# panagiotou23/model-predictive-control

Hardware: AMD Instinct MI355X
Metric: MPC solves/sec, bicycle model N=20 nx=4 nu=2, batch=65536; 1/2/4/8 GPU (higher is better)
Workload: dtype f64

## Files before the change

model_predictive_control_amd/csrc/mpc_device.hpp:

```cpp
#pragma once
#include <hip/hip_runtime.h>
#include <stdint.h>

namespace mpc {

constexpr int KIN = 0;
constexpr int PAC = 1;

struct DevCfg {
    int model, N, S, nfe, wrap_mode, clip_inputs, constr_mode, sm;
    int nx, n, m, M;
    int max_iter, max_outer, hess_heuristic, max_no_progress;
    int max_num_initial_retries, max_num_retries, max_total_num_retries, max_total_inner, max_total_evals;
    int no_spec;
    int chain;
    int all_rows;
    int no_memo;
    int no_la;
    double h;
    double v_ref;
    double w[6];
    double lf, lr, mass, inv_mass, inv_iz;
    double bf, cf, df, br, cr, dr, cm1, cm2, cr0, cr2;
    double accel, friction, max_drive, max_steer;
// ... 150 lines not shown
#pragma clang fp contract(off)
    const double kf = rint(x * 6.36619772367581382433e-01);
    double r = fma(-kf, 1.57079632679489655800e+00, x);
    r = fma(-kf, 6.12323399573676603587e-17, r);
    r = fma(-kf, -1.49738490485916983294e-33, r);
    const int q = (int)kf;
    const SinCos k = kernel_sincos(r);
    const double sn = k.s, cs = k.c;
    SinCos o;
    const bool swap = q & 1;
    const double sv = swap ? cs : sn, cv = swap ? sn : cs;
    o.s = (q & 2) ? -sv : sv;
    o.c = ((q + 1) & 2) ? -cv : cv;
    return o;
}

__device__ __forceinline__ SinCos rotate_sincos(const SinCos &a, double d)
{
#pragma clang fp contract(off)
    const SinCos k = kernel_sincos(d);
    SinCos o;
    o.s = fma(a.c, k.s, a.s * k.c);
    o.c = fma(-a.s, k.s, a.c * k.c);
    return o;
}

__device__ __noinline__ SinCos sincos_any(double x)
{
    const SinCos slow = ocml_sincos(x);
    const SinCos fast = lean_sincos(fabs(x) < 1.0e5 ? x : 0.0);
    return fabs(x) < 1.0e5 ? fast : slow;
}
__device__ __forceinline__ SinCos m_sincos(double x)
{
    if (__builtin_expect(__ballot(!(fabs(x) < 1.0e5)) == 0ull, 1)) return lean_sincos(x);
    return sincos_any(x);
}
__device__ __forceinline__ double m_sin(double x) { return m_sincos(x).s; }

__device__ __forceinline__ double atan_reduced(double r, double off_hi, double off_lo)
{
#pragma clang fp contract(off)
    const double z = r * r, w = z * z;
    double s1 = fma(w, 1.62858201153657823623e-02, 4.97687799461593236017e-02);
    s1 = fma(w, s1, 6.66107313738753120669e-02);
    s1 = fma(w, s1, 9.09088713343650656196e-02);
    s1 = fma(w, s1, 1.42857142725034663711e-01);
    s1 = z * fma(w, s1, 3.33333333333329318027e-01);
    double s2 = fma(w, -3.65315727442169155270e-02, -5.83357013379057348645e-02);
    s2 = fma(w, s2, -7.69187620504482999495e-02);
    s2 = fma(w, s2, -1.11111104054623557880e-01);
    s2 = w * fma(w, s2, -1.99999999998764832476e-01);
    return off_hi - ((r * (s1 + s2) - off_lo) - r);
}

__device__ __forceinline__ double atan_ratio(double ay, double ax)
{
#pragma clang fp contract(off)
    const bool lo = ay <= 0.41421356237309503 * ax;
    const bool hi = ay > 2.4142135623730951 * ax;
    const double num = lo ? ay : (hi ? -ax : ay - ax);
    const double den = lo ? ax : (hi ? ay : ay + ax);
    const double r = num / den;
    const double off_hi = lo ? 0.0 : (hi ? 1.57079632679489655800e+00 : 7.85398163397448278999e-01);
    const double off_lo = lo ? 0.0 : (hi ? 6.12323399573676603587e-17 : 3.06161699786838301793e-17);
    return atan_reduced(r, off_hi, off_lo);
}

MPC_ATAN_FN double m_atan(double x)
{
    const double a = fabs(x);
#ifndef MPC_ATAN_ALWAYS_DIVIDES
    if (__builtin_expect(__ballot(!(a <= 0.41421356237309503)) == 0ull, 1)) return copysign(atan_reduced(a, 0.0, 0.0), x);
#endif
    const double t = a < 1.0e300 ? atan_ratio(a, 1.0) : 1.57079632679489655800e+00;
    return x != x ? x : copysign(t, x);
}

MPC_ATAN_FN double lean_atan2(double y, double x)
{
#pragma clang fp contract(off)
    double t = atan_ratio(fabs(y), fabs(x));
    if (signbit(x)) t = 3.14159265358979311600e+00 - (t - 1.22464679914735317720e-16);
    return copysign(t, y);
}
__device__ __forceinline__ double m_atan2(double y, double x)
{
    const double ay = fabs(y), ax = fabs(x);
    const bool ok = ay < 1.0e300 && ax < 1.0e300 && (ay != 0.0 || ax != 0.0);
    if (__builtin_expect(__ballot(!ok) == 0ull, 1)) return lean_atan2(y, x);
    const double slow = ocml_atan2(y, x);
    const double fast = lean_atan2(ok ? y : 1.0, ok ? x : 1.0);
    return ok ? fast : slow;
}

template <int MODEL> struct StageInput;

template <> struct StageInput<KIN> {
    double ad;
    double beta;
    double sb_lr;
    double cb_lr;
    double dbeta;
    double mk0, mk1;
};
template <> struct StageInput<PAC> {
    double d, dl, sd, cd;
    double mk0, mk1;
};

MPC_DEV void clip_input(const DevCfg &c, double &d, double &dl, double &mk0, double &mk1)
{
    mk0 = 1.0; mk1 = 1.0;
    if (c.clip_inputs) {
        if (d > c.max_drive) { d = c.max_drive; mk0 = 0.0; }
        else if (d < -c.max_drive) { d = -c.max_drive; mk0 = 0.0; }
        if (dl > c.max_steer) { dl = c.max_steer; mk1 = 0.0; }
        else if (dl < -c.max_steer) { dl = -c.max_steer; mk1 = 0.0; }
    }
}

MPC_DEV void prep_input(const DevCfg &c, double d, double dl, StageInput<KIN> &s)
{
#pragma clang fp contract(off)
    clip_input(c, d, dl, s.mk0, s.mk1);
    const double L = c.lf + c.lr;
    const bool ok = fabs(dl) <= 0.75 && L > 0.0;
    SinCos sd = kernel_sincos(ok ? dl : 0.0);
    bool mid = false;
    if (__builtin_expect(__ballot(!ok) != 0ull, 0)) {
        mid = !ok && fabs(dl) < 1.0e5 && L > 0.0;
        const SinCos sr = lean_sincos(mid ? dl : 0.0);
        sd.s = mid ? sr.s : sd.s; sd.c = mid ? sr.c : sd.c;
    }
    const bool fast = ok || mid;
    double td = sd.s / sd.c;
    double t = c.lf * td;
    const double hyp2 = t * t + L * L;
    const double rh = 1.0 / sqrt(hyp2);
    double sb = t * rh, cb = L * rh;
    double beta;
    if (__builtin_expect(__ballot(!fast) == 0ull, 1)) beta = lean_atan2(t, L);
    else {
        const double td_s = m_tan(dl), t_s = c.lf * td_s;
        const double beta_s = m_atan2(t_s, L);
        const SinCos scb = m_sincos(beta_s);
        const double beta_f = lean_atan2(fast ? t : 0.0, fast ? L : 1.0);
        beta = fast ? beta_f : beta_s;
        td = fast ? td : td_s; t = fast ? t : t_s;
        sb = fast ? sb : scb.s; cb = fast ? cb : scb.c;
    }
    s.beta = beta;
    s.sb_lr = sb / c.lr;
    s.cb_lr = cb / c.lr;
    s.dbeta = (L / (t * t + L * L)) * c.lf * (1.0 + td * td);
    s.ad = c.accel * d;
}

MPC_DEV void prep_input(const DevCfg &c, double d, double dl, StageInput<PAC> &s)
{
    clip_input(c, d, dl, s.mk0, s.mk1);
    s.d = d; s.dl = dl;
    const SinCos sc = m_sincos(dl);
    s.sd = sc.s; s.cd = sc.c;
}

template <int MODEL> struct Lin;
template <> struct Lin<KIN> { double s, co, v; };
template <> struct Lin<PAC> {
    double sp, cp, f0, f1;
    double vx, vy, om;
    double ffy, Df, Dr;
    double vx_r1, a1_r1, vx_r2, a2_r2;
};

template <bool LIN>
MPC_DEV void rhs(const DevCfg &c, const StageInput<KIN> &u, const double (&x)[4], double (&k)[4],
                 Lin<KIN> &lin)
{
    const SinCos sc = m_sincos(x[2] + u.beta);
    const double s = sc.s, co = sc.c;
    const double v = x[3];
    k[0] = v * co;
    k[1] = v * s;
    k[2] = v * u.sb_lr;
    k[3] = u.ad - c.friction * v;
    if (LIN) { lin.s = s; lin.co = co; lin.v = v; }
}

template <bool LIN>
MPC_DEV void rhs_sc(const DevCfg &c, const StageInput<KIN> &u, const double (&x)[4], const SinCos &sc,
                    double (&k)[4], Lin<KIN> &lin)
{
#pragma clang fp contract(off)
    const double s = sc.s, co = sc.c;
    const double v = x[3];
    k[0] = v * co;
    k[1] = v * s;
    k[2] = v * u.sb_lr;
    k[3] = u.ad - c.friction * v;
    if (LIN) { lin.s = s; lin.co = co; lin.v = v; }
}

struct StepTrig { SinCos sc[4]; };
MPC_DEV void step_trig(const DevCfg &c, const StageInput<KIN> &u, const double (&x)[4], StepTrig &tr)
{
#pragma clang fp contract(off)
    const double h = c.h, hh = 0.5 * h;
    const double v1 = x[3];
    const double v2 = v1 + hh * (u.ad - c.friction * v1);
    const double v3 = v1 + hh * (u.ad - c.friction * v2);
    const double d2 = hh * (v1 * u.sb_lr), d3 = hh * (v2 * u.sb_lr), d4 = h * (v3 * u.sb_lr);
    const double th = x[2] + u.beta;
    const bool ok = fabs(d2) <= 0.75 && fabs(d3) <= 0.75 && fabs(d4) <= 0.75 && fabs(th) < 1.0e5;
    if (__builtin_expect(__ballot(!ok) == 0ull, 1)) {
        tr.sc[0] = lean_sincos(th);
        tr.sc[1] = rotate_sincos(tr.sc[0], d2);
        tr.sc[2] = rotate_sincos(tr.sc[0], d3);
        tr.sc[3] = rotate_sincos(tr.sc[0], d4);
    } else {
        const double ths = ok ? th : 0.0;
        StepTrig f;
        f.sc[0] = lean_sincos(ths);
        f.sc[1] = rotate_sincos(f.sc[0], ok ? d2 : 0.0);
        f.sc[2] = rotate_sincos(f.sc[0], ok ? d3 : 0.0);
        f.sc[3] = rotate_sincos(f.sc[0], ok ? d4 : 0.0);
        const SinCos g0 = m_sincos(th), g1 = m_sincos((x[2] + d2) + u.beta);
        const SinCos g2 = m_sincos((x[2] + d3) + u.beta), g3 = m_sincos((x[2] + d4) + u.beta);
        tr.sc[0] = ok ? f.sc[0] : g0; tr.sc[1] = ok ? f.sc[1] : g1;
        tr.sc[2] = ok ? f.sc[2] : g2; tr.sc[3] = ok ? f.sc[3] : g3;
    }
}

MPC_DEV void vjp(const DevCfg &c, const StageInput<KIN> &u, const Lin<KIN> &l, const double (&w)[4],
                 double (&yb)[4], double (&ub)[2])
{
    const double A = l.v * (w[1] * l.co - w[0] * l.s);
    yb[0] = 0.0; yb[1] = 0.0;
    yb[2] = A;
    yb[3] = w[0] * l.co + w[1] * l.s + w[2] * u.sb_lr - w[3] * c.friction;
    const double beta_b = A + w[2] * l.v * u.cb_lr;
    ub[0] += w[3] * c.accel * u.mk0;
    ub[1] += beta_b * u.dbeta * u.mk1;
}

MPC_DEV double sign_of(double v) { return (v > 0.0 ? 1.0 : 0.0) - (v < 0.0 ? 1.0 : 0.0); }

MPC_DEV void pac_assemble(const DevCfg &c, const StageInput<PAC> &u, double vx, double vy, double om, double sp,
                          double cp, double stf, double str, double (&k)[6])
{
#pragma clang fp contract(off)
    const double frx = (c.cm1 - c.cm2 * vx) * u.d - c.cr0 * sign_of(vx) - c.cr2 * vx * vx;
    const double ffy = c.df * stf;
    const double fry = c.dr * str;
    k[0] = vx * cp - vy * sp;
    k[1] = vx * sp + vy * cp;
    k[2] = om;
    k[3] = (frx - ffy * u.sd + c.mass * vy * om) * c.inv_mass;
    k[4] = (fry + ffy * u.cd - c.mass * vx * om) * c.inv_mass;
    k[5] = (ffy * c.lf * u.cd - fry * c.lr) * c.inv_iz;
}

template <bool LIN>
MPC_DEV void rhs(const DevCfg &c, const StageInput<PAC> &u, const double (&x)[6], double (&k)[6],
                 Lin<PAC> &lin)
{
    const double vx = x[3], vy = x[4], om = x[5];
    const double a1 = om * c.lf + vy;
    const double a2 = om * c.lr - vy;
    const double fa1 = fabs(a1), fa2 = fabs(a2), fvx = fabs(vx);
    const bool ok = fabs(x[2]) < 1.0e5 && fa1 < 1.0e300 && fa2 < 1.0e300 && fvx < 1.0e300 &&
                    (fvx != 0.0 || (fa1 != 0.0 && fa2 != 0.0)) && fabs(u.dl) < 1.0e5 &&
                    fabs(c.cf) < 6.0e4 && fabs(c.cr) < 6.0e4;
    double sp, cp, af, ar, stf, ctf, str, ctr;
    if (__builtin_expect(__ballot(!ok) == 0ull, 1)) {
        const SinCos scp = lean_sincos(x[2]);
        sp = scp.s; cp = scp.c;
        af = u.dl - lean_atan2(a1, vx);
        ar = lean_atan2(a2, vx);
        const SinCos a = lean_sincos(c.cf * m_atan(c.bf * af)), b = lean_sincos(c.cr * m_atan(c.br * ar));
        stf = a.s; ctf = a.c; str = b.s; ctr = b.c;
    } else {
        const SinCos scp = m_sincos(x[2]);
        sp = scp.s; cp = scp.c;
        af = u.dl - m_atan2(a1, vx);
        ar = m_atan2(a2, vx);
        const SinCos a = m_sincos(c.cf * m_atan(c.bf * af)), b = m_sincos(c.cr * m_atan(c.br * ar));
        stf = a.s; ctf = a.c; str = b.s; ctr = b.c;
    }
    const double ffy = c.df * stf;
    pac_assemble(c, u, vx, vy, om, sp, cp, stf, str, k);
    if (LIN) {
        lin.sp = sp; lin.cp = cp; lin.f0 = k[0]; lin.f1 = k[1];
        lin.vx = vx; lin.vy = vy; lin.om = om;
        lin.ffy = ffy;
        const double baf = c.bf * af, bar = c.br * ar;
        lin.Df = c.df * ctf * c.cf * c.bf / (1.0 + baf * baf);
        lin.Dr = c.dr * ctr * c.cr * c.br / (1.0 + bar * bar);
        const double ir1 = 1.0 / (a1 * a1 + vx * vx), ir2 = 1.0 / (a2 * a2 + vx * vx);
        lin.vx_r1 = vx * ir1; lin.a1_r1 = a1 * ir1;
        lin.vx_r2 = vx * ir2; lin.a2_r2 = a2 * ir2;
    }
}

MPC_DEV void vjp(const DevCfg &c, const StageInput<PAC> &u, const Lin<PAC> &l, const double (&w)[6],
                 double (&yb)[6], double (&ub)[2])
// ... 621 lines not shown
```

model_predictive_control_amd/csrc/mpc_eval.hpp:

```cpp
#pragma once
#include "mpc_solver.hpp"

#ifndef MPC_K1B_WAVES_PAC
#define MPC_K1B_WAVES_PAC 1
#endif
#ifndef MPC_QUAD_WAVES
#define MPC_QUAD_WAVES 2
#endif

namespace mpc {

struct SlotMap {
    int nG, nC, gpad, nblk_g, nblk;
    __device__ SlotMap(const int *counts, int nG_imm, int nC_imm)
    {
        nG = counts ? counts[0] : nG_imm;
        nC = counts ? counts[1] : nC_imm;
        gpad = (nG + 63) & ~63;
        nblk_g = gpad >> 6;
        nblk = nblk_g + ((nC + 63) >> 6);
    }
};

template <int MODEL, bool PA = false>
__global__ void __launch_bounds__(64, 2)
rollout_kernel(const DevCfg c, const WsArg<PA> w, const int *__restrict__ lists,
               const int *__restrict__ counts, int nG_imm, int nC_imm)
{
    constexpr int NX = ModelDim<MODEL>::NX;
    extern __shared__ double lds[];
    double *tile = lds;
    int *s_agent = (int *)(lds + 64 * (c.n + 1));
    const SlotMap sm(counts, nG_imm, nC_imm);
    const int sb = blockIdx.x;
    if (sb >= sm.nblk) return;
    const int lane = threadIdx.x;
    const bool is_g = sb < sm.nblk_g;
    const int uslot = sb * 64 + lane;
    const int kslot = is_g ? uslot : uslot - sm.gpad;
    const bool active = kslot < (is_g ? sm.nG : sm.nC);
    const int *list = counts ? (is_g ? lists : lists + w.Ls) : nullptr;
    const int raw = active ? (list ? list[kslot] : kslot) : -1;
    const int a = raw < 0 ? -1 : raw & AGENT_MASK;
    const int n = c.n, N = c.N, ld = n + 1;
    s_agent[lane] = raw;
    w.agent_of[uslot] = raw;
    __syncthreads();
    const int total = 64 * n;
    for (int base = 0; base < total; base += 64 * 8) {
        double v[8];
        int off[8];
#pragma unroll
        for (int u = 0; u < 8; u++) {
            const int idx = base + u * 64 + lane;
            const int r = idx / n, j = idx - r * n;
            const int ar = idx < total ? s_agent[r] : -1;
            off[u] = ar >= 0 ? r * ld + j : -1;
            v[u] = ar >= 0 ? ((ar & CH2_BIT) ? w.xe2 : w.xe)[(size_t)(ar & AGENT_MASK) * n + j] : 0.0;
        }
#pragma unroll
        for (int u = 0; u < 8; u++) if (off[u] >= 0) tile[off[u]] = v[u];
    }
    __syncthreads();
    if (!active) return;
    DevCfg cm_;
    if constexpr (PA) { cm_ = c; agent_cfg(cm_, w.ptab, w.pidx, a); }
    const DevCfg &cm = PA ? cm_ : c;
    const size_t St = (size_t)w.St;
    const double *urow = tile + lane * ld;
    double x[NX];
#pragma unroll
    for (int i = 0; i < NX; i++) { x[i] = w.x0[(size_t)a * NX + i]; w.trajx[(size_t)i * St + uslot] = x[i]; }
    for (int k = 0; k < N; k++) {
        const double d = urow[2 * k], dl = urow[2 * k + 1];
        w.useq[(size_t)(2 * k) * St + uslot] = d;
        w.useq[(size_t)(2 * k + 1) * St + uslot] = dl;
        StageInput<MODEL> u;
        prep_input(cm, d, dl, u);
        stage_forward<MODEL>(cm, u, x);
#pragma unroll
        for (int i = 0; i < NX; i++) w.trajx[(size_t)((k + 1) * NX + i) * St + uslot] = x[i];
    }
}

#ifndef MPC_K1A_WAVES
#define MPC_K1A_WAVES 3
#endif
template <class Put>
__device__ __forceinline__ void kin_wide_rollout(const DevCfg &c, const double (&x0)[4], double d, double dl, int lane, Put put);
template <bool PA = false>
__global__ void __launch_bounds__(64, MPC_K1A_WAVES)
rollout_pair_kernel(const DevCfg c, const WsArg<PA> w, const int *__restrict__ lists,
                    const int *__restrict__ counts, int nG_imm, int nC_imm)
{
#pragma clang fp contract(off)
#if MPC_DEV_STAMP == 1
    DevStamp stamp(blockIdx.x);
#endif
    constexpr int RPB = 32;
    extern __shared__ double lds[];
    const SlotMap sm(counts, nG_imm, nC_imm);
    const int lane = threadIdx.x, q = lane >> 1, half = lane & 1;
    const int uslot = blockIdx.x * RPB + q;
    const int nslots = sm.nblk * 64;
    const bool is_g = uslot < sm.gpad;
    const int kslot = is_g ? uslot : uslot - sm.gpad;
    const bool active = uslot < nslots && kslot < (is_g ? sm.nG : sm.nC);
    const int *list = counts ? (is_g ? lists : lists + w.Ls) : nullptr;
    const int raw = active ? (list ? list[kslot] : kslot) : -1;
    const int n = c.n, N = c.N, ld = n + 1;
    if (half == 0 && uslot < nslots) w.agent_of[uslot] = raw;
    if (__ballot(active) == 0ull) return;
    {
        const double *__restrict__ row = ((raw & CH2_BIT) ? w.xe2 : w.xe) + (size_t)(raw & AGENT_MASK) * n;
        for (int j0 = half; j0 < n; j0 += 16) {
            double v[8];
#pragma unroll
            for (int t = 0; t < 8; t++) v[t] = active && j0 + 2 * t < n ? row[j0 + 2 * t] : 0.0;
#pragma unroll
            for (int t = 0; t < 8; t++) if (j0 + 2 * t < n) lds[q * ld + j0 + 2 * t] = v[t];
        }
    }
    __builtin_amdgcn_wave_barrier();
    const int a = active ? raw & AGENT_MASK : 0;
    DevCfg cm_;
    if constexpr (PA) { cm_ = c; if (active) agent_cfg(cm_, w.ptab, w.pidx, a); }
    const DevCfg &cm = PA ? cm_ : c;
    const size_t St = (size_t)w.St;
    const double *urow = lds + q * ld;
    double x[4];
#pragma unroll
    for (int i = 0; i < 4; i++) x[i] = active ? w.x0[(size_t)a * 4 + i] : 0.0;
    bool redo = false;
    auto put = [&](int k) {
        if (!active || redo) return;
        w.trajx[(size_t)(k * 4 + 2 * half) * St + uslot] = half ? x[2] : x[0];
        w.trajx[(size_t)(k * 4 + 2 * half + 1) * St + uslot] = half ? x[3] : x[1];
    };
    put(0);
    auto stage = [&](int k, const StageInput<KIN> &u) {
        const double d = urow[2 * k], dl = urow[2 * k + 1];
        if (active) w.useq[(size_t)(2 * k + half) * St + uslot] = half ? dl : d;
        redo = redo || !kin4_in_range(cm, u, x);
#if MPC_DEV_STAMP == 1
        if (__ballot(redo) != 0ull) stamp.nfall++;
#endif
        double ph = x[2], v = x[3];
        KinRK k0, k1, k2, k3;
        const double ph0 = ph; kin_rk(cm, u, v, k0); kin_next(cm, k0, ph, v);
        const double ph1 = ph; kin_rk(cm, u, v, k1); kin_next(cm, k1, ph, v);
        const double ph2 = ph; kin_rk(cm, u, v, k2); kin_next(cm, k2, ph, v);
        const double ph3 = ph; kin_rk(cm, u, v, k3); kin_next(cm, k3, ph, v);
        KinRK ka, kb;
        ka.v1 = half ? k2.v1 : k0.v1; ka.v2 = half ? k2.v2 : k0.v2; ka.v3 = half ? k2.v3 : k0.v3; ka.v4 = half ? k2.v4 : k0.v4;
        ka.kp1 = half ? k2.kp1 : k0.kp1; ka.kp2 = half ? k2.kp2 : k0.kp2; ka.kp3 = half ? k2.kp3 : k0.kp3;
        kb.v1 = half ? k3.v1 : k1.v1; kb.v2 = half ? k3.v2 : k1.v2; kb.v3 = half ? k3.v3 : k1.v3; kb.v4 = half ? k3.v4 : k1.v4;
        kb.kp1 = half ? k3.kp1 : k1.kp1; kb.kp2 = half ? k3.kp2 : k1.kp2; kb.kp3 = half ? k3.kp3 : k1.kp3;
        double dxa, dya, dxb, dyb;
        kin_increment(cm, u, half ? ph2 : ph0, ka, !redo, dxa, dya);
        kin_increment(cm, u, half ? ph3 : ph1, kb, !redo, dxb, dyb);
        const double oxa = dpp_xchg<0xB1>(dxa), oya = dpp_xchg<0xB1>(dya);
        const double oxb = dpp_xchg<0xB1>(dxb), oyb = dpp_xchg<0xB1>(dyb);
        double px = x[0], py = x[1];
        px = px + dxa; py = py + dya;
        px = px + dxb; py = py + dyb;
        px = px + oxa; py = py + oya;
        px = px + oxb; py = py + oyb;
        x[0] = px; x[1] = py; x[2] = ph; x[3] = v;
        put(k + 1);
    };
    for (int k = 0; k < N; k += 2) {
        const int km = min(k + half, N - 1);
        StageInput<KIN> um, up;
#if MPC_DEV_STAMP == 1
        if (__ballot(!(fabs(urow[2 * km + 1]) <= 0.75)) != 0ull) stamp.nmid++;
        if (__ballot(!(fabs(urow[2 * km + 1]) < 1.0e5)) != 0ull) stamp.nslow++;
#endif
        prep_input(cm, urow[2 * km], urow[2 * km + 1], um);
        up.ad = dpp_xchg<0xB1>(um.ad); up.beta = dpp_xchg<0xB1>(um.beta);
        up.sb_lr = dpp_xchg<0xB1>(um.sb_lr); up.cb_lr = dpp_xchg<0xB1>(um.cb_lr);
        up.dbeta = dpp_xchg<0xB1>(um.dbeta); up.mk0 = dpp_xchg<0xB1>(um.mk0); up.mk1 = dpp_xchg<0xB1>(um.mk1);
        StageInput<KIN> ua, ub;
        ua.ad = half ? up.ad : um.ad; ua.beta = half ? up.beta : um.beta; ua.sb_lr = half ? up.sb_lr : um.sb_lr;
        ua.cb_lr = half ? up.cb_lr : um.cb_lr; ua.dbeta = half ? up.dbeta : um.dbeta;
        ua.mk0 = half ? up.mk0 : um.mk0; ua.mk1 = half ? up.mk1 : um.mk1;
        ub.ad = half ? um.ad : up.ad; ub.beta = half ? um.beta : up.beta; ub.sb_lr = half ? um.sb_lr : up.sb_lr;
        ub.cb_lr = half ? um.cb_lr : up.cb_lr; ub.dbeta = half ? um.dbeta : up.dbeta;
        ub.mk0 = half ? um.mk0 : up.mk0; ub.mk1 = half ? um.mk1 : up.mk1;
        stage(k, ua);
        if (k + 1 < N) stage(k + 1, ub);
    }
    unsigned long long todo = __ballot(redo && active && half == 0);
    while (todo != 0ull) {
        const int l0 = (int)__builtin_ctzll(todo);
        todo &= todo - 1ull;
        const int aq = __builtin_amdgcn_readlane(raw, l0) & AGENT_MASK;
        const int uq = blockIdx.x * RPB + (l0 >> 1);
        const double *uro = lds + (l0 >> 1) * ld;
        const bool stage_lane = lane < N;
        const double dq = stage_lane ? uro[2 * lane] : 0.0, dlq = stage_lane ? uro[2 * lane + 1] : 0.0;
        double xq[4];
#pragma unroll
        for (int i = 0; i < 4; i++) xq[i] = w.x0[(size_t)aq * 4 + i];
        double *const tj = w.trajx + uq;
        if constexpr (PA) {
            DevCfg cq = c;
            agent_cfg_uniform(cq, w.ptab, w.pidx, aq);
            kin_wide_rollout(cq, xq, dq, dlq, lane, [=](int k, int i, double v) { tj[(size_t)(k * 4 + i) * St] = v; });
        } else
        kin_wide_rollout(c, xq, dq, dlq, lane, [=](int k, int i, double v) { tj[(size_t)(k * 4 + i) * St] = v; });
    }
}


template <bool PA = false>
__global__ void __launch_bounds__(64, MPC_QUAD_WAVES)
rollout_quad_kernel(const DevCfg c, const WsArg<PA> w, const int *__restrict__ lists,
                    const int *__restrict__ counts, int nG_imm, int nC_imm)
{
    constexpr int NX = 6, RPB = 16;
    extern __shared__ double lds[];
#if MPC_DEV_STAMP == 4
    DevStamp stamp(blockIdx.x);
#endif
    const SlotMap sm(counts, nG_imm, nC_imm);
    const int lane = threadIdx.x, q = lane >> 2, role = lane & 3;
    const int uslot = blockIdx.x * RPB + q;
    const int nslots = sm.nblk * 64;
    const bool is_g = uslot < sm.gpad;
    const int kslot = is_g ? uslot : uslot - sm.gpad;
    const bool active = uslot < nslots && kslot < (is_g ? sm.nG : sm.nC);
    const int *list = counts ? (is_g ? lists : lists + w.Ls) : nullptr;
    const int raw = active ? (list ? list[kslot] : kslot) : -1;
    const int n = c.n, N = c.N, ld = n + 1;
    if (role == 0 && uslot < nslots) w.agent_of[uslot] = raw;
    if (active) {
        const double *__restrict__ row = ((raw & CH2_BIT) ? w.xe2 : w.xe) + (size_t)(raw & AGENT_MASK) * n;
        for (int j0 = role; j0 < n; j0 += 32) {
            double v[8];
#pragma unroll
            for (int t = 0; t < 8; t++) v[t] = j0 + 4 * t < n ? row[j0 + 4 * t] : 0.0;
#pragma unroll
            for (int t = 0; t < 8; t++) if (j0 + 4 * t < n) lds[q * ld + j0 + 4 * t] = v[t];
        }
    }
    __builtin_amdgcn_wave_barrier();
    if (!active) return;
    const int a = raw & AGENT_MASK;
    DevCfg cm_;
    if constexpr (PA) { cm_ = c; agent_cfg(cm_, w.ptab, w.pidx, a); }
    const DevCfg &cm = PA ? cm_ : c;
    const size_t St = (size_t)w.St;
    const double *urow = lds + q * ld;
    double x[NX];
#pragma unroll
    for (int i = 0; i < NX; i++) x[i] = w.x0[(size_t)a * NX + i];
    auto put = [&](int k) {
        w.trajx[(size_t)(k * NX + role) * St + uslot] = role == 0 ? x[0] : role == 1 ? x[1] : role == 2 ? x[2] : x[3];
        if (role < 2) w.trajx[(size_t)(k * NX + 4 + role) * St + uslot] = role == 0 ? x[4] : x[5];
    };
    put(0);
    for (int k = 0; k < N; k++) {
        const double d = urow[2 * k], dl = urow[2 * k + 1];
        if (role == 0) w.useq[(size_t)(2 * k) * St + uslot] = d;
        if (role == 1) w.useq[(size_t)(2 * k + 1) * St + uslot] = dl;
        StageInput<PAC> u;
        prep_input(cm, d, dl, u);
#if MPC_DEV_STAMP == 4
        {
            bool fin = true;
#pragma unroll
            for (int i = 0; i < NX; i++) fin = fin && fabs(x[i]) < 1.0e300;
            const bool inr = fabs(x[2]) < 1.0e5 && fabs(dl) < 1.0e5 && (x[3] != 0.0 || (x[5] * c.lf + x[4] != 0.0 && x[5] * c.lr - x[4] != 0.0));
            if (__ballot(!fin) != 0ull) stamp.nfall++;
            if (__ballot(fin && !inr) != 0ull) stamp.nmid++;
            if (__ballot(!fin) != 0ull && k == 0) stamp.nslow++;
        }
#endif
        stage_forward_quad(cm, u, x, role);
        put(k + 1);
    }
}

template <class Put>
__device__ __forceinline__ void kin_wide_rollout(const DevCfg &c, const double (&x0)[4], double d, double dl, int lane, Put put)
{
    const int N = c.N;
    const bool stage_lane = lane < N;
    StageInput<KIN> u;
    prep_input(c, d, dl, u);
    if (lane == 0) {
#pragma unroll
        for (int i = 0; i < 4; i++) put(0, i, x0[i]);
    }
    double ph = x0[2], v = x0[3];
    constexpr int PASS = 4;
    double cph[PASS] = {0.0, 0.0, 0.0, 0.0}, cv[PASS] = {0.0, 0.0, 0.0, 0.0}, eph = 0.0, ev = 0.0;
    int gen = 0;
    bool anygen = false;
#pragma unroll
    for (int p = 0; p < PASS; p++) {
        const int k1 = N < 16 * (p + 1) ? N : 16 * (p + 1);
        for (int k = 16 * p; k < k1; k++) {
            StageInput<KIN> uk;
            uk.ad = rdlane(u.ad, k); uk.beta = rdlane(u.beta, k); uk.sb_lr = rdlane(u.sb_lr, k);
            const double xs[4] = {0.0, 0.0, ph, v};
            const bool inr = __ballot(!kin4_in_range(c, uk, xs)) == 0ull;
            anygen = anygen || !inr;
#pragma unroll
            for (int j = 0; j < 4; j++) {
                if (lane == ((4 * k + j) & 63)) { cph[p] = ph; cv[p] = v; gen |= inr ? 0 : 1 << p; }
                KinRK kr;
                if (inr) { kin_rk(c, uk, v, kr); kin_next(c, kr, ph, v); }
                else { kin_gen_rk(c, uk, v, kr); kin_gen_next(c, kr, ph, v); }
            }
            if (lane == k) { eph = ph; ev = v; }
        }
    }
    double dx[PASS] = {0.0, 0.0, 0.0, 0.0}, dy[PASS] = {0.0, 0.0, 0.0, 0.0};
#pragma unroll
    for (int p = 0; p < PASS; p++) {
        const int s = 64 * p + lane;
        if (64 * p >= 4 * N) break;
        const int k = (s >> 2) < N ? (s >> 2) : N - 1;
        StageInput<KIN> uk;
        uk.ad = __shfl(u.ad, k); uk.beta = __shfl(u.beta, k); uk.sb_lr = __shfl(u.sb_lr, k);
        const bool g = ((gen >> p) & 1) != 0 && (s >> 2) < N;
        KinRK kr;
        kin_rk(c, uk, cv[p], kr);
        kin_increment(c, uk, cph[p], kr, !g, dx[p], dy[p]);
        if (anygen) {
            double gx, gy;
            kin_gen_rk(c, uk, g ? cv[p] : 0.0, kr);
            kin_gen_increment(c, uk, g ? cph[p] : 0.0, g ? cv[p] : 0.0, kr, gx, gy);
            dx[p] = g ? gx : dx[p]; dy[p] = g ? gy : dy[p];
        }
    }
    double px = x0[0], py = x0[1], epx = 0.0, epy = 0.0;
#pragma unroll
    for (int p = 0; p < PASS; p++) {
        const int k0 = 16 * p, k1 = N < 16 * (p + 1) ? N : 16 * (p + 1);
        for (int k = k0; k < k1; k++) {
#pragma clang fp contract(off)
#pragma unroll
            for (int j = 0; j < 4; j++) {
                px = px + rdlane(dx[p], (4 * k + j) & 63);
                py = py + rdlane(dy[p], (4 * k + j) & 63);
            }
            if (lane == k) { epx = px; epy = py; }
        }
    }
    if (stage_lane) { put(lane + 1, 0, epx); put(lane + 1, 1, epy); put(lane + 1, 2, eph); put(lane + 1, 3, ev); }
}

template <bool PA = false>
__global__ void __launch_bounds__(256)
rollout_wide_kernel(const DevCfg c, const WsArg<PA> w, const int *__restrict__ lists,
                    const int *__restrict__ counts)
{
    const SlotMap sm(counts, 0, 0);
    const int lane = threadIdx.x & 63, wv = threadIdx.x >> 6;
    const int uslot = blockIdx.x * 4 + wv;
    if (uslot >= sm.nblk * 64) return;
// ... 396 lines not shown
```

model_predictive_control_amd/csrc/mpc_solver.hpp:

```cpp
#pragma once
#include "mpc_device.hpp"
#include <float.h>

namespace mpc {

constexpr int REC = 64;
enum {
    R_PSI, R_L, R_GAMMA, R_PHI, R_PSIXH, R_PP, R_GP, R_TAU, R_PSIN, R_LN, R_GAMMAN, R_PSIXHN, R_GPN,
    R_PPN, R_SIGPP, R_EPS, R_HN2, R_HFD, R_GAMMA_TOP, R_DELTA, R_RHO, R_EPS_OLD, R_NE1, R_PS_EPS,
    R_OUT_EPS, R_OUT_DELTA, R_PSI_OUT, R_PSIE,
    R_PHASE, R_K, R_LIDX, R_LFULL, R_NOPROG, R_NJ, R_OUTER, R_FIRST, R_INITRED, R_PENRED,
    R_INNER_TOT, R_INNER_FAIL, R_STATUS, R_NEVALS, R_MAXIT, R_OVERWRITE, R_FALLBACK, R_PS_STATUS,
    R_PS_ITERS, R_OUT_OF_ITER, R_NGRAD, R_LBROWS, R_SPEC, R_SPEC_GAMMA, R_NSPEC, R_NSPEC_USED, R_NCOST,
    R_RUN_MINEPS, R_RUN_EV0, R_MEMO_STATUS, R_MEMO_ITERS, R_MEMO_EVALS, R_MEMO_MINEPS, R_MEMO_EPS,
    R_LA_EVALS, R_LA_HITS, R_USED
};
static_assert(R_USED <= REC, "record too small");
__host__ __device__ constexpr bool rec_is_int(int s)
{
    return (s >= R_PHASE && s <= R_OUT_OF_ITER) || s == R_SPEC || (s >= R_RUN_EV0 && s <= R_MEMO_EVALS);
}
__device__ __forceinline__ double rec_int(int k) { return __hiloint2double(0x43300000, k); }
__device__ __forceinline__ int rec_int_of(double v) { return __double2loint(v); }

enum Phase {
    PH_DONE = 0,
    PH_W_INIT_H = 1, PH_W_INIT_X, PH_W_DL, PH_W_HEUR, PH_W_HESS, PH_W_LS_G, PH_W_LS_C,
    PH_OUTER_BEGIN = 16, PH_TOP, PH_AFTER_DL, PH_LS_INIT, PH_LS_TRIAL, PH_INNER_EXIT
};
enum { ST_UNKNOWN = 0, ST_CONVERGED = 1, ST_MAXTIME = 2, ST_MAXITER = 3, ST_NOTFINITE = 4,
       ST_NOPROGRESS = 5 };
enum { REQ_NONE = 0, REQ_GRAD = 1, REQ_COST = 2, REQ_SPEC = 4,
       REQ_CHAIN = 8 };
constexpr int CH2_BIT = 1 << 30;
constexpr int CHAIN_BIT = 1 << 29;
constexpr int AGENT_MASK = CHAIN_BIT - 1;
constexpr int PH_MASK = 63;
__device__ __forceinline__ int chain_tag(int par) { return 64 * (1 + par); }

struct Workspace {
    const double *x0;
    double *xo;
    double *xk, *gk, *q, *xn, *xe, *ge;
    double *xe2, *ge2;
    double *S, *Y;
    double *y;
    double *Sig, *Sig_old, *e1, *e2, *yhx, *yhxn, *yhe;
    double *rec;
    int *lists;
    int *counts;
    unsigned long long *totals;
    int *solo_ctr;
    double *trajx;
    double *useq;
    double *stage_L;
    double *jac;
    int *agent_of;
    const double *cl;
    const int *cl_index;
    NearTab near;
    double *psi_direct;
    double *ws_xe, *ws_ge, *ws_yhe, *ws_Sig;
    int B, Bp;
    int St;
    int Ls;
};
struct WorkspacePA : Workspace {
    const double *ptab;
    const int *pidx;
};
struct BoxTab {
    const double *btab;
    const int *bidx;
};
struct ConTab {
    const double *ctab;
    const int *cidx;
};
__device__ __forceinline__ void agent_con(DevCfg &c, const ConTab &t, int a) { agent_con(c, t.ctab, t.cidx, a); }
__device__ __forceinline__ void agent_con_uniform(DevCfg &c, const ConTab &t, int a) { agent_con_uniform(c, t.ctab, t.cidx, a); }
struct DiscTab {
    const double *dtab;
    const int *didx;
};
__device__ __forceinline__ StageDiscs stage_discs(const DiscTab &t, int a, int k, int N)
{
    const double *__restrict__ r = t.dtab + ((size_t)t.didx[a] * N + k) * (3 * NDISC);
    StageDiscs s;
#pragma unroll
    for (int i = 0; i < 3 * NDISC; i++) s.v[i] = r[i];
    return s;
}
__device__ __forceinline__ StageDiscs stage_discs_uniform(const DiscTab &t, int a, int k, int N)
{
    const int row = __builtin_amdgcn_readfirstlane(t.didx[a]);
    const double *__restrict__ r = t.dtab + (size_t)row * N * (3 * NDISC) + (size_t)k * (3 * NDISC);
    StageDiscs s;
#pragma unroll
    for (int i = 0; i < 3 * NDISC; i++) s.v[i] = r[i];
    return s;
}
struct RateTab {
    const double *rtab;
    const int *ridx;
};
template <class Prev, class Next>
__device__ __forceinline__ StageRate stage_rate_from(const double *__restrict__ r, int k, int N, Prev prev_of, Next next_of)
{
    StageRate s;
    s.w[0] = r[0]; s.w[1] = r[1];
    s.last = k == N - 1;
    if (k == 0) { s.prev[0] = r[2]; s.prev[1] = r[3]; }
    else { s.prev[0] = prev_of(0); s.prev[1] = prev_of(1); }
    if (s.last) { s.next[0] = 0.0; s.next[1] = 0.0; }
    else { s.next[0] = next_of(0); s.next[1] = next_of(1); }
    return s;
}
__device__ __forceinline__ StageRate stage_rate(const RateTab &t, int a, int k, int N, const double *__restrict__ useq_slot, size_t St)
{
    return stage_rate_from(t.rtab + (size_t)t.ridx[a] * NRATE, k, N,
                           [=](int i) { return useq_slot[(size_t)(2 * (k - 1) + i) * St]; },
                           [=](int i) { return useq_slot[(size_t)(2 * (k + 1) + i) * St]; });
}
__device__ __forceinline__ StageRate stage_rate_uniform(const RateTab &t, int a, int k, int N, const double *__restrict__ row)
{
    const int ri = __builtin_amdgcn_readfirstlane(t.ridx[a]);
    return stage_rate_from(t.rtab + (size_t)ri * NRATE, k, N, [=](int i) { return row[2 * (k - 1) + i]; },
                           [=](int i) { return row[2 * (k + 1) + i]; });
}
struct FieldTab {
    const double *ftab;
    const int *fidx;
};
__device__ __forceinline__ StageField stage_field(const FieldTab &t, int a, int k, int N)
{
    return StageField{t.ftab + ((size_t)t.fidx[a] * N + k) * (NFIELD * NFSRC)};
}
__device__ __forceinline__ StageField stage_field_uniform(const FieldTab &t, int a, int k, int N)
{
    const int row = __builtin_amdgcn_readfirstlane(t.fidx[a]);
    return StageField{t.ftab + (size_t)row * N * (NFIELD * NFSRC) + (size_t)k * (NFIELD * NFSRC)};
}
template <class A, class B> struct SameTab { static constexpr bool v = false; };
template <class A> struct SameTab<A, A> { static constexpr bool v = true; };
template <class X, class... T> constexpr bool has_tab = (SameTab<X, T>::v || ... || false);
template <class X, class T0, class... T>
__device__ __forceinline__ const X &pack_get(const T0 &t0, const T &...t)
{
    if constexpr (SameTab<X, T0>::v) return t0;
    else return pack_get<X>(t...);
}
template <bool PA> struct WsArgT { using type = Workspace; };
template <> struct WsArgT<true> { using type = WorkspacePA; };
template <bool PA> using WsArg = typename WsArgT<PA>::type;

struct KernArgs {
    static constexpr size_t W_OFF = (sizeof(DevCfg) + alignof(Workspace) - 1) / alignof(Workspace) * alignof(Workspace);
    const __attribute__((address_space(4))) char *p;
    __device__ __forceinline__ explicit KernArgs(bool on = true) : p(nullptr)
    {
        if (!on) return;
        p = (const __attribute__((address_space(4))) char *)__builtin_amdgcn_kernarg_segment_ptr();
        asm volatile("" : "+s"(p));
    }
    __device__ __forceinline__ const DevCfg &c() const { return *(const DevCfg *)p; }
    __device__ __forceinline__ const Workspace &w() const { return *(const Workspace *)(p + W_OFF); }
    static constexpr size_t B_OFF = (W_OFF + sizeof(Workspace) + alignof(BoxTab) - 1) / alignof(BoxTab) * alignof(BoxTab);
    __device__ __forceinline__ const BoxTab &box() const { return *(const BoxTab *)(p + B_OFF); }
    static_assert(sizeof(ConTab) == sizeof(BoxTab) && alignof(ConTab) == alignof(BoxTab), "one layout for the two table arguments");
    __device__ __forceinline__ const ConTab &con(bool behind_box) const { return *(const ConTab *)(p + B_OFF + (behind_box ? sizeof(BoxTab) : 0)); }
    __device__ __forceinline__ int *con_tail(bool behind_box, int i) const
    {
        return *(int *const *)(p + B_OFF + (behind_box ? sizeof(BoxTab) : 0) + sizeof(ConTab) + i * sizeof(int *));
    }
};

#ifdef MPC_DEV_STAMP
constexpr int DEV_STAMPS = 65536;
__device__ long long g_dev_stamps[4 * DEV_STAMPS];
struct DevStamp {
    long long t0; int idx; int nfall = 0, nmid = 0, nslow = 0;
    __device__ DevStamp(int i) : t0(__builtin_amdgcn_s_memrealtime()), idx(i) {}
    __device__ ~DevStamp()
    {
        if ((threadIdx.x & 63) == 0 && idx < DEV_STAMPS) {
            g_dev_stamps[4 * idx] = t0; g_dev_stamps[4 * idx + 1] = __builtin_amdgcn_s_memrealtime();
            g_dev_stamps[4 * idx + 2] = __builtin_amdgcn_s_getreg((4 << 0) | (0 << 6) | (31 << 11));
            g_dev_stamps[4 * idx + 3] = (__builtin_amdgcn_s_getreg((20 << 0) | (0 << 6) | (31 << 11)) & 15)
                                        | ((long long)nfall << 8) | ((long long)nmid << 16) | ((long long)nslow << 24);
        }
    }
};
#endif
__device__ __forceinline__ double rdlane(double v, int l)
{
    const int lo = __builtin_amdgcn_readlane(__double2loint(v), l);
    const int hi = __builtin_amdgcn_readlane(__double2hiint(v), l);
    return __hiloint2double(hi, lo);
}
template <int CTRL>
__device__ __forceinline__ double dpp_xchg(double v)
{
    int lo = __double2loint(v), hi = __double2hiint(v);
    lo = __builtin_amdgcn_update_dpp(0, lo, CTRL, 0xf, 0xf, false);
    hi = __builtin_amdgcn_update_dpp(0, hi, CTRL, 0xf, 0xf, false);
    return __hiloint2double(hi, lo);
}
__device__ __forceinline__ double row_sum16(double v)
{
    v += dpp_xchg<0xB1>(v);
    v += dpp_xchg<0x4E>(v);
    v += dpp_xchg<0x141>(v);
    v += dpp_xchg<0x140>(v);
    return v;
}
template <int NROWS = 4>
__device__ __forceinline__ double cross_rows(double v)
{
    if (NROWS <= 2) return rdlane(v, 0) + rdlane(v, 16);
    if (NROWS == 3) return (rdlane(v, 0) + rdlane(v, 16)) + rdlane(v, 32);
    return (rdlane(v, 0) + rdlane(v, 16)) + (rdlane(v, 32) + rdlane(v, 48));
}
__device__ __forceinline__ double wave_sum(double v)
{
    v = row_sum16(v);
    return cross_rows<4>(v);
}
__device__ __forceinline__ double fast_rcp(double x)
{
    double r = __builtin_amdgcn_rcp(x);
    r = fma(r, fma(-x, r, 1.0), r);
    r = fma(r, fma(-x, r, 1.0), r);
    return r;
}
__device__ __forceinline__ double fd_step(double xx)
{
#pragma clang fp contract(off)
    return cbrt(DBL_EPSILON) * (1.0 + sqrt(xx));
}
__device__ __forceinline__ void wave_sum2(double &a, double &b)
{
    a = row_sum16(a); b = row_sum16(b);
    a = cross_rows<4>(a); b = cross_rows<4>(b);
}
__device__ __forceinline__ double wave_sum_n(double v, int n)
{
    v = row_sum16(v);
    return n <= 32 ? cross_rows<2>(v) : n <= 48 ? cross_rows<3>(v) : cross_rows<4>(v);
}
__device__ __forceinline__ void wave_sum2_n(double &a, double &b, int n)
{
    a = row_sum16(a); b = row_sum16(b);
    if (n <= 32) { a = cross_rows<2>(a); b = cross_rows<2>(b); }
    else if (n <= 48) { a = cross_rows<3>(a); b = cross_rows<3>(b); }
    else { a = cross_rows<4>(a); b = cross_rows<4>(b); }
}
__device__ __forceinline__ void wave_sum3(double &a, double &b, double &c)
{
    a = row_sum16(a); b = row_sum16(b); c = row_sum16(c);
    a = (rdlane(a, 0) + rdlane(a, 16)) + (rdlane(a, 32) + rdlane(a, 48));
    b = (rdlane(b, 0) + rdlane(b, 16)) + (rdlane(b, 32) + rdlane(b, 48));
    c = (rdlane(c, 0) + rdlane(c, 16)) + (rdlane(c, 32) + rdlane(c, 48));
}
__device__ __forceinline__ double wave_max(double v)
{
    v = fmax(v, dpp_xchg<0xB1>(v)); v = fmax(v, dpp_xchg<0x4E>(v));
    v = fmax(v, dpp_xchg<0x141>(v)); v = fmax(v, dpp_xchg<0x140>(v));
    return fmax(fmax(rdlane(v, 0), rdlane(v, 16)), fmax(rdlane(v, 32), rdlane(v, 48)));
}

__device__ __forceinline__ double rfl(double v)
{
    const int lo = __builtin_amdgcn_readfirstlane(__double2loint(v));
    const int hi = __builtin_amdgcn_readfirstlane(__double2hiint(v));
    return __hiloint2double(hi, lo);
}
struct RecD {
    double &rv; const int &lane; const int slot;
    __device__ __forceinline__ operator double() const { return rdlane(rv, slot); }
    __device__ __forceinline__ RecD &operator=(double x) { rv = lane == slot ? x : rv; return *this; }
    __device__ __forceinline__ RecD &operator=(const RecD &o) { return *this = (double)o; }
    __device__ __forceinline__ RecD &operator*=(double x) { return *this = (double)*this * x; }
    __device__ __forceinline__ RecD &operator/=(double x) { return *this = (double)*this / x; }
};
struct RecI {
    double &rv; const int &lane; const int slot;
    __device__ __forceinline__ operator int() const { return __builtin_amdgcn_readlane(__double2loint(rv), slot); }
    __device__ __forceinline__ RecI &operator=(int x)
    {
        const int lo = __double2loint(rv);
        rv = __hiloint2double(__double2hiint(rv), lane == slot ? x : lo);
        return *this;
    }
    __device__ __forceinline__ RecI &operator=(const RecI &o) { return *this = (int)o; }
    __device__ __forceinline__ RecI &operator+=(int x) { return *this = (int)*this + x; }
    __device__ __forceinline__ RecI &operator|=(int x) { return *this = (int)*this | x; }
    __device__ __forceinline__ RecI &operator++(int) { return *this = (int)*this + 1; }
};

struct LocI {
    int v; const int slot;
    __device__ __forceinline__ LocI(double rv, int s) : v(__builtin_amdgcn_readlane(__double2loint(rv), s)), slot(s) {}
    __device__ __forceinline__ operator int() const { return v; }
    __device__ __forceinline__ LocI &operator=(int x) { v = x; return *this; }
    __device__ __forceinline__ LocI &operator++(int) { v = v + 1; return *this; }
    __device__ __forceinline__ void put(double &rv, int lane) const
    { rv = __hiloint2double(__double2hiint(rv), lane == slot ? v : __double2loint(rv)); }
};

template <int NE> struct Row { double v[NE]; };

template <int NE>
__device__ __forceinline__ Row<NE> ldrow(const double *__restrict__ p, int n, int lane)
{
    Row<NE> r;
#pragma unroll
    for (int e = 0; e < NE; e++) { const int j = lane + 64 * e; r.v[e] = j < n ? p[j] : 0.0; }
    return r;
}
// ... 1084 lines not shown
```

Measured before the change: 508,900.

## Cut register pressure in paired-lane kinematic rollout via DPP broadcast and kernarg reloads

Reworks the two-lane kinematic rollout. The per-lane stage-input swap-and-select is replaced with DPP quad broadcasts, and input preparation uses a leaner prep_input_fast that always takes the fast atan2 path and marks slow cases with NaN. The four RK stage structs are collapsed into one reused struct, with the needed stages recomputed from saved velocities. Trajectory and input stores use incrementing pointers instead of per-call index math, and the fallback path reloads config and workspace from kernarg memory so fewer values stay live. The aim is lower VGPR use and fewer selects, at the cost of extra RK recomputation and a changed handling of out-of-range steering inputs.

```diff
diff --git a/model_predictive_control_amd/csrc/mpc_device.hpp b/model_predictive_control_amd/csrc/mpc_device.hpp
--- a/model_predictive_control_amd/csrc/mpc_device.hpp
+++ b/model_predictive_control_amd/csrc/mpc_device.hpp
@@ -326,6 +326,32 @@
     }
     s.beta = beta;
     s.sb_lr = sb / c.lr;
+    s.cb_lr = cb / c.lr;
+    s.dbeta = (L / (t * t + L * L)) * c.lf * (1.0 + td * td);
+    s.ad = c.accel * d;
+}
+
+MPC_DEV void prep_input_fast(const DevCfg &c, double d, double dl, StageInput<KIN> &s)
+{
+#pragma clang fp contract(off)
+    clip_input(c, d, dl, s.mk0, s.mk1);
+    const double L = c.lf + c.lr;
+    const bool ok = fabs(dl) <= 0.75 && L > 0.0;
+    SinCos sd = kernel_sincos(ok ? dl : 0.0);
+    bool mid = false;
+    if (__builtin_expect(__ballot(!ok) != 0ull, 0)) {
+        mid = !ok && fabs(dl) < 1.0e5 && L > 0.0;
+        const SinCos sr = lean_sincos(mid ? dl : 0.0);
+        sd.s = mid ? sr.s : sd.s; sd.c = mid ? sr.c : sd.c;
+    }
+    const bool fast = ok || mid;
+    const double td = sd.s / sd.c;
+    const double t = c.lf * td;
+    const double hyp2 = t * t + L * L;
+    const double rh = 1.0 / sqrt(hyp2);
+    const double sb = t * rh, cb = L * rh;
+    s.beta = lean_atan2(t, L);
+    s.sb_lr = fast ? sb / c.lr : __builtin_nan("");
     s.cb_lr = cb / c.lr;
     s.dbeta = (L / (t * t + L * L)) * c.lf * (1.0 + td * td);
     s.ad = c.accel * d;
diff --git a/model_predictive_control_amd/csrc/mpc_eval.hpp b/model_predictive_control_amd/csrc/mpc_eval.hpp
--- a/model_predictive_control_amd/csrc/mpc_eval.hpp
+++ b/model_predictive_control_amd/csrc/mpc_eval.hpp
@@ -132,33 +132,36 @@
 #pragma unroll
     for (int i = 0; i < 4; i++) x[i] = active ? w.x0[(size_t)a * 4 + i] : 0.0;
     bool redo = false;
-    auto put = [&](int k) {
-        if (!active || redo) return;
-        w.trajx[(size_t)(k * 4 + 2 * half) * St + uslot] = half ? x[2] : x[0];
-        w.trajx[(size_t)(k * 4 + 2 * half + 1) * St + uslot] = half ? x[3] : x[1];
+    const bool lo = active && half == 0, hi = active && half != 0;
+    double *tk = w.trajx + (size_t)blockIdx.x * RPB;
+    double *uk = w.useq + (size_t)blockIdx.x * RPB;
+    auto put = [&]() {
+        if (lo && !redo) { tk[q] = x[0]; tk[St + q] = x[1]; }
+        if (hi && !redo) { tk[2 * St + q] = x[2]; tk[3 * St + q] = x[3]; }
+        tk += 4 * St;
     };
-    put(0);
+    put();
     auto stage = [&](int k, const StageInput<KIN> &u) {
         const double d = urow[2 * k], dl = urow[2 * k + 1];
-        if (active) w.useq[(size_t)(2 * k + half) * St + uslot] = half ? dl : d;
+        if (lo) uk[q] = d;
+        if (hi) uk[St + q] = dl;
+        uk += 2 * St;
         redo = redo || !kin4_in_range(cm, u, x);
 #if MPC_DEV_STAMP == 1
         if (__ballot(redo) != 0ull) stamp.nfall++;
 #endif
         double ph = x[2], v = x[3];
-        KinRK k0, k1, k2, k3;
-        const double ph0 = ph; kin_rk(cm, u, v, k0); kin_next(cm, k0, ph, v);
-        const double ph1 = ph; kin_rk(cm, u, v, k1); kin_next(cm, k1, ph, v);
-        const double ph2 = ph; kin_rk(cm, u, v, k2); kin_next(cm, k2, ph, v);
-        const double ph3 = ph; kin_rk(cm, u, v, k3); kin_next(cm, k3, ph, v);
+        KinRK kk;
+        const double ph0 = ph, v0 = v; kin_rk(cm, u, v, kk); kin_next(cm, kk, ph, v);
+        const double ph1 = ph, v1 = v; kin_rk(cm, u, v, kk); kin_next(cm, kk, ph, v);
+        const double ph2 = ph, v2 = v; kin_rk(cm, u, v, kk); kin_next(cm, kk, ph, v);
+        const double ph3 = ph, v3 = v; kin_rk(cm, u, v, kk); kin_next(cm, kk, ph, v);
         KinRK ka, kb;
-        ka.v1 = half ? k2.v1 : k0.v1; ka.v2 = half ? k2.v2 : k0.v2; ka.v3 = half ? k2.v3 : k0.v3; ka.v4 = half ? k2.v4 : k0.v4;
-        ka.kp1 = half ? k2.kp1 : k0.kp1; ka.kp2 = half ? k2.kp2 : k0.kp2; ka.kp3 = half ? k2.kp3 : k0.kp3;
-        kb.v1 = half ? k3.v1 : k1.v1; kb.v2 = half ? k3.v2 : k1.v2; kb.v3 = half ? k3.v3 : k1.v3; kb.v4 = half ? k3.v4 : k1.v4;
-        kb.kp1 = half ? k3.kp1 : k1.kp1; kb.kp2 = half ? k3.kp2 : k1.kp2; kb.kp3 = half ? k3.kp3 : k1.kp3;
+        kin_rk(cm, u, half ? v2 : v0, ka);
+        kin_rk(cm, u, half ? v3 : v1, kb);
         double dxa, dya, dxb, dyb;
-        kin_increment(cm, u, half ? ph2 : ph0, ka, !redo, dxa, dya);
-        kin_increment(cm, u, half ? ph3 : ph1, kb, !redo, dxb, dyb);
+        kin_increment(cm, u, half ? ph2 : ph0, ka, true, dxa, dya);
+        kin_increment(cm, u, half ? ph3 : ph1, kb, true, dxb, dyb);
         const double oxa = dpp_xchg<0xB1>(dxa), oya = dpp_xchg<0xB1>(dya);
         const double oxb = dpp_xchg<0xB1>(dxb), oyb = dpp_xchg<0xB1>(dyb);
         double px = x[0], py = x[1];
@@ -167,48 +170,53 @@
         px = px + oxa; py = py + oya;
         px = px + oxb; py = py + oyb;
         x[0] = px; x[1] = py; x[2] = ph; x[3] = v;
-        put(k + 1);
+        put();
     };
     for (int k = 0; k < N; k += 2) {
         const int km = min(k + half, N - 1);
-        StageInput<KIN> um, up;
+        StageInput<KIN> um;
 #if MPC_DEV_STAMP == 1
         if (__ballot(!(fabs(urow[2 * km + 1]) <= 0.75)) != 0ull) stamp.nmid++;
         if (__ballot(!(fabs(urow[2 * km + 1]) < 1.0e5)) != 0ull) stamp.nslow++;
 #endif
-        prep_input(cm, urow[2 * km], urow[2 * km + 1], um);
-        up.ad = dpp_xchg<0xB1>(um.ad); up.beta = dpp_xchg<0xB1>(um.beta);
-        up.sb_lr = dpp_xchg<0xB1>(um.sb_lr); up.cb_lr = dpp_xchg<0xB1>(um.cb_lr);
-        up.dbeta = dpp_xchg<0xB1>(um.dbeta); up.mk0 = dpp_xchg<0xB1>(um.mk0); up.mk1 = dpp_xchg<0xB1>(um.mk1);
+        const KernArgs kl(!PA);
+        const DevCfg &cp = PA ? cm : kl.c();
+        prep_input_fast(cp, urow[2 * km], urow[2 * km + 1], um);
         StageInput<KIN> ua, ub;
-        ua.ad = half ? up.ad : um.ad; ua.beta = half ? up.beta : um.beta; ua.sb_lr = half ? up.sb_lr : um.sb_lr;
-        ua.cb_lr = half ? up.cb_lr : um.cb_lr; ua.dbeta = half ? up.dbeta : um.dbeta;
-        ua.mk0 = half ? up.mk0 : um.mk0; ua.mk1 = half ? up.mk1 : um.mk1;
-        ub.ad = half ? um.ad : up.ad; ub.beta = half ? um.beta : up.beta; ub.sb_lr = half ? um.sb_lr : up.sb_lr;
-        ub.cb_lr = half ? um.cb_lr : up.cb_lr; ub.dbeta = half ? um.dbeta : up.dbeta;
-        ub.mk0 = half ? um.mk0 : up.mk0; ub.mk1 = half ? um.mk1 : up.mk1;
+        ua.ad = dpp_xchg<0xA0>(um.ad); ua.beta = dpp_xchg<0xA0>(um.beta); ua.sb_lr = dpp_xchg<0xA0>(um.sb_lr);
+        ua.cb_lr = dpp_xchg<0xA0>(um.cb_lr); ua.dbeta = dpp_xchg<0xA0>(um.dbeta);
+        ua.mk0 = dpp_xchg<0xA0>(um.mk0); ua.mk1 = dpp_xchg<0xA0>(um.mk1);
+        ub.ad = dpp_xchg<0xF5>(um.ad); ub.beta = dpp_xchg<0xF5>(um.beta); ub.sb_lr = dpp_xchg<0xF5>(um.sb_lr);
+        ub.cb_lr = dpp_xchg<0xF5>(um.cb_lr); ub.dbeta = dpp_xchg<0xF5>(um.dbeta);
+        ub.mk0 = dpp_xchg<0xF5>(um.mk0); ub.mk1 = dpp_xchg<0xF5>(um.mk1);
         stage(k, ua);
         if (k + 1 < N) stage(k + 1, ub);
     }
     unsigned long long todo = __ballot(redo && active && half == 0);
+    if (__builtin_expect(todo == 0ull, 0)) return;
     while (todo != 0ull) {
+        const KernArgs kr;
+        const DevCfg &cr = kr.c();
+        const WsArg<PA> &wr = kr.ws<PA>();
         const int l0 = (int)__builtin_ctzll(todo);
         todo &= todo - 1ull;
         const int aq = __builtin_amdgcn_readlane(raw, l0) & AGENT_MASK;
-        const int uq = blockIdx.x * RPB + (l0 >> 1);
-        const double *uro = lds + (l0 >> 1) * ld;
-        const bool stage_lane = lane < N;
+        const int uq = __builtin_amdgcn_readlane(uslot, l0);
+        const int Nr = cr.N;
+        const double *uro = lds + (l0 >> 1) * (cr.n + 1);
+        const bool stage_lane = lane < Nr;
         const double dq = stage_lane ? uro[2 * lane] : 0.0, dlq = stage_lane ? uro[2 * lane + 1] : 0.0;
         double xq[4];
 #pragma unroll
-        for (int i = 0; i < 4; i++) xq[i] = w.x0[(size_t)aq * 4 + i];
-        double *const tj = w.trajx + uq;
+        for (int i = 0; i < 4; i++) xq[i] = wr.x0[(size_t)aq * 4 + i];
+        double *const tj = wr.trajx + uq;
+        const size_t Sr = (size_t)wr.St;
         if constexpr (PA) {
-            DevCfg cq = c;
-            agent_cfg_uniform(cq, w.ptab, w.pidx, aq);
-            kin_wide_rollout(cq, xq, dq, dlq, lane, [=](int k, int i, double v) { tj[(size_t)(k * 4 + i) * St] = v; });
+            DevCfg cq = cr;
+            agent_cfg_uniform(cq, wr.ptab, wr.pidx, aq);
+            kin_wide_rollout(cq, xq, dq, dlq, lane, [=](int k, int i, double v) { tj[(size_t)(k * 4 + i) * Sr] = v; });
         } else
-        kin_wide_rollout(c, xq, dq, dlq, lane, [=](int k, int i, double v) { tj[(size_t)(k * 4 + i) * St] = v; });
+        kin_wide_rollout(cr, xq, dq, dlq, lane, [=](int k, int i, double v) { tj[(size_t)(k * 4 + i) * Sr] = v; });
     }
 }
 
diff --git a/model_predictive_control_amd/csrc/mpc_solver.hpp b/model_predictive_control_amd/csrc/mpc_solver.hpp
--- a/model_predictive_control_amd/csrc/mpc_solver.hpp
+++ b/model_predictive_control_amd/csrc/mpc_solver.hpp
@@ -155,6 +155,7 @@
 template <bool PA> using WsArg = typename WsArgT<PA>::type;
 
 struct KernArgs {
+    static_assert(alignof(WorkspacePA) == alignof(Workspace), "one offset for the two workspace arguments");
     static constexpr size_t W_OFF = (sizeof(DevCfg) + alignof(Workspace) - 1) / alignof(Workspace) * alignof(Workspace);
     const __attribute__((address_space(4))) char *p;
     __device__ __forceinline__ explicit KernArgs(bool on = true) : p(nullptr)
@@ -165,6 +166,7 @@
     }
     __device__ __forceinline__ const DevCfg &c() const { return *(const DevCfg *)p; }
     __device__ __forceinline__ const Workspace &w() const { return *(const Workspace *)(p + W_OFF); }
+    template <bool PA> __device__ __forceinline__ const WsArg<PA> &ws() const { return *(const WsArg<PA> *)(p + W_OFF); }
     static constexpr size_t B_OFF = (W_OFF + sizeof(Workspace) + alignof(BoxTab) - 1) / alignof(BoxTab) * alignof(BoxTab);
     __device__ __forceinline__ const BoxTab &box() const { return *(const BoxTab *)(p + B_OFF); }
     static_assert(sizeof(ConTab) == sizeof(BoxTab) && alignof(ConTab) == alignof(BoxTab), "one layout for the two table arguments");
```

Measured after the change: 512,800, median of 6. About the same (+0.8%).
